# leejet/stable-diffusion.cpp

Measured on AMD Instinct MI355X. Metric: denoise it/s (image-iterations/s: cond+uncond UNet forwards per image per step), higher is better.
Workload: dtype f16; 1 GPU; sd15 UNet 512x512, cfg 7 (cond+uncond), f16 weights, batch 8/GPU, Euler-A step; global_batch=8, flash_attn=True, hip_graph=1, cfg_pair_in_one_graph=True, device_resident_sampler=True

## Files before the change

include/ggml-mi355x.h:

```cpp
#ifndef GGML_MI355X_H
#define GGML_MI355X_H

#include "ggml-abi.h"

#ifdef __cplusplus
extern "C" {
#endif

#define GGML_MI355X_API __attribute__((visibility("default")))

GGML_MI355X_API ggml_backend_reg_t ggml_backend_init(void);
GGML_MI355X_API int ggml_backend_score(void);
GGML_MI355X_API ggml_backend_reg_t ggml_backend_mi355x_reg(void);
GGML_MI355X_API int ggml_backend_mi355x_get_device_count(void);

struct ggml_backend_mi355x_stats {
    int64_t graphs_computed;
    int64_t plans_built;
    int64_t nodes_seen;
    int64_t kernels_planned;
    int64_t kernels_launched;
    int64_t fused_conv;
    int64_t fused_conv_bounced;
    int64_t fused_linear;
// ... 34 lines not shown
    int64_t fused_concat_gn;
    int64_t fused_conv_scale;
    int64_t view_graphs;
    int64_t plans_evicted;
    int64_t hoisted_mod_linears;
    int64_t view_external_nodes;
    int64_t qinloop_linears;
    int64_t flash_out_alias;
    int64_t flash_slice_images;
    int64_t flash_short_launches;
    int64_t flash_qb2_launches;
    int64_t flash_mslot_launches;
    int64_t flash_generic_launches;
    int64_t fused_gn_epilogue;
    int64_t fused_tile_merge;
};
GGML_MI355X_API void ggml_backend_mi355x_get_stats(struct ggml_backend_mi355x_stats* out);
GGML_MI355X_API int ggml_backend_mi355x_resolve_enums(const char* (*op_name)(int), const char* (*unary_op_name)(int), const char* (*type_name)(int));
GGML_MI355X_API const char* ggml_backend_mi355x_enum_status(void);
GGML_MI355X_API void ggml_backend_mi355x_get_enum_maps(uint8_t* ops256, uint8_t* unary256);
struct ggml_backend_mi355x_kernel_timing {
    char kernel[96];
    int64_t launches;
    double total_ms;
    double total_flops;
    double total_bytes;
    int32_t bound;
    int32_t family;
};
GGML_MI355X_API void ggml_backend_mi355x_kernel_timing_enable(int enable);
// ... 29 lines not shown
```

stable-diffusion.cpp_amd/__init__.py:

```python
from __future__ import annotations

import ctypes as C
import os
from pathlib import Path

import numpy as np

PKG_DIR = Path(__file__).resolve().parent
ROOT = PKG_DIR.parent
LIB_DIR = PKG_DIR / "lib"
HOST_LIB = Path(os.environ.get("SDCPP_HOST_LIB", str(LIB_DIR / "libsdcpp-host.so")))
BACKEND_LIB = Path(os.environ.get("SDCPP_BACKEND_LIB", str(LIB_DIR / "libggml-mi355x.so")))

F32, F16, Q4_0, Q8_0, I32, BF16 = 0, 1, 2, 8, 26, 30
TYPE_SIZE = {F32: 4, F16: 2, BF16: 2, I32: 4}

SD15, SDXL, SD15_TINY, SDXL_TINY, SD35_LARGE, SD35_TINY, FLUX_DEV, FLUX_TINY, SD35_WIDE2, FLUX_WIDE1, SD3M_TINY, SD35_WIDE8, FLUX_WIDE8 = 0, 1, 2, 3, 4, 5, 6, 7, 8, 9, 10, 11, 12
PAIR_EXCHANGE_FN = C.CFUNCTYPE(C.c_bool, C.c_void_p, C.c_int64, C.c_void_p, C.c_void_p)
EVAL_CALLBACK_FN = C.CFUNCTYPE(C.c_bool, C.c_void_p, C.c_bool, C.c_void_p)
EULER, EULER_A, HEUN, DPM2, DPMPP2S_A, DPMPP2M, DPMPP2Mv2, IPNDM, IPNDM_V, LCM, DDIM_TRAILING = range(11)
TCD, RES_MULTISTEP, RES_2S, ER_SDE, EULER_CFG_PP, EULER_A_CFG_PP, EULER_GE, DPMPP2M_SDE, DPMPP2M_SDE_BT, LMS = range(11, 21)
SAMPLE_METHOD_DEFAULT = 21
SCHED_DISCRETE, SCHED_KARRAS, SCHED_EXPONENTIAL, SCHED_AYS, SCHED_GITS, SCHED_SGM_UNIFORM, SCHED_SIMPLE, SCHED_SMOOTHSTEP, SCHED_KL_OPTIMAL, SCHED_LCM = range(10)
SCHED_BONG_TANGENT, SCHED_FLUX, SCHED_BETA, SCHEDULER_DEFAULT = 10, 14, 15, 16
# ... 337 lines not shown
    _loaded_plugins.add(p)


def load_mi355x_backend() -> None:
    if not BACKEND_LIB.exists():
        raise EngineError(f"{BACKEND_LIB} missing — the HIP backend was not built")
    load_backend(BACKEND_LIB)
    names = devices()
    if not any(n.upper().startswith("MI355X") for n in names):
        raise EngineError(f"libggml-mi355x.so loaded but exposes no MI355X device (devices: {names}); is a gfx950 GPU visible?")


_BACKEND_STAT_FIELDS = ("graphs_computed plans_built nodes_seen kernels_planned kernels_launched fused_conv fused_conv_bounced fused_linear "
                        "fused_norm fused_geglu fused_attention generic_matmul swizzled_weight_bytes graph_replays fused_linear_geglu "
                        "split_k_gemms head_major_gemms fused_modulate fused_gate fused_gelu fused_rope fused_concat_heads qgemv_linears fused_chan_add fused_proj_tokens gemm_attention fused_q16 split_k_inlaunch qgemm16_linears fgemv_linears fused_presilu fused_sibling_linears hoisted_kv_linears window_convs hoisted_emb_linears fused_rows16 fused_joint_qkv jit_images fused_cat_rows16 fused_gn_stats fused_ln_reduce redirect_fallbacks fused_concat_gn fused_conv_scale view_graphs plans_evicted hoisted_mod_linears view_external_nodes qinloop_linears flash_out_alias flash_slice_images "
                        "flash_short_launches flash_qb2_launches flash_mslot_launches flash_generic_launches fused_gn_epilogue fused_tile_merge").split()


class BackendStats(C.Structure):
    _fields_ = [(n, C.c_int64) for n in _BACKEND_STAT_FIELDS]


_backend_cdll = None


def _backend() -> C.CDLL:
    global _backend_cdll
    if _backend_cdll is None:
        load_mi355x_backend()
        _backend_cdll = C.CDLL(str(BACKEND_LIB))
        _backend_cdll.ggml_backend_mi355x_get_stats.argtypes = [C.POINTER(BackendStats)]
# ... 740 lines not shown
```

stable-diffusion.cpp_amd/csrc/backend/planner.cpp:

```cpp
#include "planner.h"

#include <atomic>
#include <cstddef>
#include <cstdio>
#include <cstdlib>
#include <cstring>
#include <functional>
#include <memory>
#include <mutex>
#include <string>
#include <algorithm>
#include <map>
#include <unordered_map>
#include <unordered_set>
#include <vector>

#include "kernels.h"
#include "ktime.h"

namespace mi355x {

static uint8_t g_opmap[256];
static uint8_t g_unmap[256];
static bool g_opmap_init = [] {
// ... 94 lines not shown
    return true;
}
void planner_get_op_maps(uint8_t* ops256, uint8_t* unary256) {
    if (ops256) memcpy(ops256, g_opmap, 256);
    if (unary256) memcpy(unary256, g_unmap, 256);
}

namespace {

constexpr size_t N_STATS = sizeof(ggml_backend_mi355x_stats) / sizeof(int64_t);
static_assert(N_STATS * sizeof(int64_t) == sizeof(ggml_backend_mi355x_stats), "ggml_backend_mi355x_stats: int64_t fields only");
std::atomic<int64_t> g_stat_counters[N_STATS];
#define STAT(field) g_stat_counters[offsetof(ggml_backend_mi355x_stats, field) / sizeof(int64_t)]

struct Options {
    std::atomic<int> fusion{1}, mfma_gemm{1}, hip_graph{1}, flash_pattern{1}, fuse_modulate{1}, fuse_gate{1}, fuse_gelu{1}, fuse_rope{1}, fuse_concat_heads{1}, qgemv{1}, fuse_chan_add{1}, fuse_proj_tokens{1}, fuse_q16{1}, qgemm16{1}, fgemv{1}, fuse_siblings{1}, hoist_kv{1}, hoist_emb{1}, fuse_rows16{0}, fuse_cat_rows16{1}, fuse_joint_qkv{1}, jit_qimages{4096}, fuse_gn_stats{1}, fuse_ln_reduce{1}, relax_res_overlap{1}, fuse_split_gelu{1}, fuse_concat_gn{1}, fuse_gn_tokens{1}, fuse_linear_nchw{1}, fuse_conv_scale{1}, ignore_use_counts{0}, plan_cache_cap{512}, hoist_mod{1}, fuse_flash_slices{1}, fuse_act_pack{1}, fuse_gn_epilogue{1}, fuse_tile_merge{1};
} g_opt;

using Step = std::function<void(hipStream_t)>;

struct Plan {
    int n_nodes = 0;
    uint64_t check = 0;
    size_t arena_needed = 0;
    std::vector<Step> steps;
    hipGraphExec_t graph_exec = nullptr;
    bool graph_failed         = false;
    int64_t runs              = 0;
    uint64_t last_use         = 0;
};

// ... 299 lines not shown
        Epilogue ep;
        int hd, hH, hL;
    };
    std::vector<HmLaunch> hm_group;
    std::unordered_map<const ggml_tensor*, size_t> moved;
    struct MovedEmb {
        size_t off;
        int64_t ld, M, N;
    };
    std::unordered_map<const ggml_tensor*, MovedEmb> moved_emb;
    struct GnPre {
        size_t off;
        const float *w, *b;
        int groups;
        float eps;
    };
    std::unordered_map<const ggml_tensor*, GnPre> gn_pre;
    std::unordered_map<const ggml_tensor*, size_t> gn_rec;
    struct LnPre {
        size_t off;
        const float *w, *b;
        float eps;
    };
    std::unordered_map<const ggml_tensor*, LnPre> ln_pre;
    struct Cat16 {
        size_t off;
        int64_t ld;
        bool written[2];
    };
    struct Cat16Part {
// ... 209 lines not shown
                    mul = sc;
                } else {
                    if (!(xop(cn) == GGML_OP_IM2COL && cn->src[1] == gi.node(k) && conv_im2col_fast_ok(gi, c))) return false;
                    if (n_real > 0 && mul != 1.f) return false;
                }
            } else {
                if (!(xop(cn) == GGML_OP_MUL_MAT && strip_reshape(cn->src[1]) == t && linear_fast_ok(cn))) return false;
            }
            ++n_real;
        }
    }
    if (mul_out) *mul_out = mul;
    return n_real > 0;
}

bool linear_fast_ok(const ggml_tensor* n) {
    const ggml_tensor* w = n->src[0];
    const ggml_tensor* x = n->src[1];
    if (!g_opt.mfma_gemm) return false;
    if (!is_static_weight(w) || !is_f32(x) || !is_f32(n)) return false;
    if (!(w->type == GGML_TYPE_F16 || w->type == GGML_TYPE_F32 || w->type == GGML_TYPE_BF16 || w->type == GGML_TYPE_Q8_0 || w->type == GGML_TYPE_Q4_0)) return false;
    if (w->ne[2] != 1 || w->ne[3] != 1 || !contig(w)) return false;
    if (x->nb[0] != 4 || x->ne[0] % 4 != 0 || x->nb[1] % 16 != 0 || !aligned16(x->data)) return false;
    if (x->ne[2] > 1 && x->nb[2] != x->nb[1] * (size_t)x->ne[1]) {
        if (x->ne[3] != 1 || x->nb[2] % 16 != 0) return false;
    }
    if (x->ne[3] > 1 && x->nb[3] != x->nb[2] * (size_t)x->ne[2]) return false;
    if (!contig(n)) return false;
    return true;
}
// ... 1043 lines not shown
        int r = gi.sole(last);
        if (r >= 0 && !gi.done[r] && xop(gi.node(r)) == GGML_OP_ADD && gi.only_noops_between(last, r, chain)) {
            const ggml_tensor* a     = gi.node(r);
            const ggml_tensor* other = a->src[0] == gi.node(last) ? a->src[1] : (a->src[1] == gi.node(last) ? a->src[0] : nullptr);
            if (other && is_f32(other) && contig(other) && contig(a) && ggml_abi_same_shape(other, a) && ggml_abi_same_shape(out, a) && gi.idx(other) < i &&
                (other->data == a->data || !overlaps(a->data, ob, other->data, ob))) {
                ep.residual = (const float*)other->data;
                chain.push_back(r);
                last = r;
            }
        }
    }
    float* final_dst = (float*)gi.node(last)->data;
    const int ks = KW, st_ = s0, pd = p0;
    Builder::GnPre gnp{0, nullptr, nullptr, 0, 0.f};
    if (g_opt.fuse_gn_stats && token_major_out < 0) {
        const ggml_tensor* res = gi.node(last);
        for (int k : gi.consumers[last]) {
            if (gnp.groups) break;
            const ggml_tensor* g = gi.node(k);
            if (xop(g) != GGML_OP_GROUP_NORM || g->src[0] != res || gi.done[k]) continue;
            const int j1 = gi.sole(k);
            if (j1 < 0 || xop(gi.node(j1)) != GGML_OP_MUL || gi.node(j1)->src[0] != g || !bias_like_chan(gi.node(j1)->src[1], OC)) break;
            const int j2 = gi.sole(j1);
            if (j2 < 0 || xop(gi.node(j2)) != GGML_OP_ADD || gi.node(j2)->src[0] != gi.node(j1) || !bias_like_chan(gi.node(j2)->src[1], OC)) break;
            const int64_t ohw = res->ne[0] * res->ne[1];
            if (!splitk_reduce_gn_supported(ohw, OC, N, g->op_params[0])) break;
            gnp = Builder::GnPre{0, (const float*)gi.node(j1)->src[1]->data, (const float*)gi.node(j2)->src[1]->data, g->op_params[0], ggml_abi_op_param_f32(g, 1)};
        }
    }
    const bool rec_want = g_opt.fuse_gn_epilogue && g_opt.fusion && token_major_out < 0 && feeds_group_norm(gi, last);
    auto gn_register = [&](int S) -> bool {
        if (S <= 1 || !gnp.groups) return false;
        if ((((uintptr_t)final_dst | (uintptr_t)ep.residual) & 15) != 0) return false;
        gnp.off                    = B.alloc((size_t)N * OC * 4 * 2);
        B.gn_pre[gi.node(last)]    = gnp;
        STAT(fused_gn_stats)++;
        return true;
    };
    auto gn_fill = [](Epilogue& e, const Builder::GnPre& g, char* arena, int64_t nc) {
        e.gn_scale  = (float*)(arena + g.off);
        e.gn_shift  = e.gn_scale + nc;
        e.gn_w      = g.w;
        e.gn_b      = g.b;
        e.gn_groups = g.groups;
        e.gn_eps    = g.eps;
    };
    const bool ups_in = B.ups.find(xs) != B.ups.end();
    const int w3S     = (token_major_out < 0) ? conv3w_plan(x->ne[0], x->ne[1], IC, N, OC, ks, st_, ups_in) : 0;
    const void* swz   = get_swz_conv(B.P, ker, s, w3S > 0);
    if (!swz) return false;
    const ggml_tensor* src = xs;
    bool upscale           = false;
    auto ui                = B.ups.find(xs);
    if (ui != B.ups.end()) {
        src     = ui->second;
        upscale = true;
    }
    const int64_t SW = src->ne[0], SH = src->ne[1];
    auto it = B.packed.find(src);
    if (it != B.packed.end() && it->second.nhwc && it->second.mul != pre_mul) {
// ... 77 lines not shown
    const size_t off = pk.off;
    const float* tp  = (const float*)t->data;
    B.emit([=](hipStream_t st) { launch_pack_rows_f16(st, P->arena + off, tp, N * HW, C, C); });
    B.packed[xr] = pk;
    return true;
}

bool plan_group_norm(Builder& B, int i, hipStream_t, std::vector<int>& chain) {
    GInfo& gi            = B.gi;
    const ggml_tensor* n = gi.node(i);
    const ggml_tensor* x = n->src[0];
    if (!is_f32(x) || !contig(x) || !contig(n)) return false;
    const int groups = n->op_params[0];
    const float eps  = ggml_abi_op_param_f32(n, 1);
    const int64_t hw = x->ne[0] * x->ne[1], C = x->ne[2], N = x->ne[3];
    const float *w = nullptr, *b = nullptr;
    bool silu = false;
    chain.push_back(i);
    int last = i;
    if (g_opt.fusion) {
        int j1 = gi.sole(i);
        if (j1 >= 0 && xop(gi.node(j1)) == GGML_OP_MUL && gi.node(j1)->src[0] == n && bias_like_chan(gi.node(j1)->src[1], C) && gi.node(j1)->data == n->data &&
            gi.only_noops_between(i, j1, chain)) {
            int j2 = gi.sole(j1);
            if (j2 >= 0 && xop(gi.node(j2)) == GGML_OP_ADD && gi.node(j2)->src[0] == gi.node(j1) && bias_like_chan(gi.node(j2)->src[1], C) &&
                gi.node(j2)->data == n->data && gi.only_noops_between(j1, j2, chain)) {
                w = (const float*)gi.node(j1)->src[1]->data;
                b = (const float*)gi.node(j2)->src[1]->data;
                chain.push_back(j1);
                chain.push_back(j2);
                last   = j2;
                int j3 = gi.sole(j2);
                if (j3 >= 0 && xop(gi.node(j3)) == GGML_OP_UNARY && xunary(gi.node(j3)) == GGML_UNARY_OP_SILU && gi.node(j3)->data == n->data &&
                    gi.only_noops_between(j2, j3, chain)) {
                    silu = true;
                    chain.push_back(j3);
                    last = j3;
                }
            }
        }
    }
    float* dst      = (float*)n->data;
    const float* xp = (const float*)x->data;
    int tok_cont = -1;
    if (g_opt.fusion && g_opt.fuse_gn_tokens && w && !silu) {
        const int jp = gi.sole(last);
        const ggml_tensor* pt = jp >= 0 ? gi.node(jp) : nullptr;
        if (pt && xop(pt) == GGML_OP_PERMUTE && pt->src[0] == gi.node(last) && pt->op_params[0] == 1 && pt->op_params[1] == 2 && pt->op_params[2] == 0 && pt->op_params[3] == 3) {
            const int jc = gi.sole(jp);
            const ggml_tensor* ct = jc >= 0 ? gi.node(jc) : nullptr;
            if (ct && xop(ct) == GGML_OP_CONT && ct->src[0] == pt && is_f32(ct) && contig(ct) && ct->ne[0] == C && !(ct->flags & GGML_TENSOR_FLAG_OUTPUT) && all_consumers_gemm16(gi, jc, false)) {
                std::vector<int> c2 = chain;
                c2.push_back(jp);
                c2.push_back(jc);
                if (gi.only_noops_between(last, jc, c2)) tok_cont = jc;
            }
        }
    }
    if (tok_cont >= 0) {
        Planner* P       = B.P;
        const auto pre   = B.gn_pre.find(x);
        const bool have  = pre != B.gn_pre.end() && pre->second.w == w && pre->second.b == b && pre->second.groups == groups && pre->second.eps == eps;
        const size_t so  = have ? pre->second.off : B.alloc((size_t)N * C * 4 * 2);
        const size_t off = B.alloc((size_t)N * hw * rup64(C) * 2);
        const auto rec   = B.gn_rec.find(x);
        const bool byrec = !have && g_opt.fuse_gn_epilogue && rec != B.gn_rec.end();
        const size_t ro  = byrec ? rec->second : 0;
        const int gsp    = (have || byrec) ? 0 : gn_stats_split(hw, C, N, groups);
        const size_t po  = gsp ? B.alloc((size_t)N * groups * gsp * 2 * 4) : 0;
        if (byrec) STAT(fused_gn_epilogue)++;
        B.emit([=](hipStream_t st) {
            float* sc = (float*)(P->arena + so);
            float* sh = sc + N * C;
            if (byrec) launch_gn_finalize(st, sc, sh, (const GnRec*)(P->arena + ro), nullptr, hw, C, C, N, groups, eps, w, b);
            else if (!have) launch_gn_stats(st, sc, sh, xp, hw, C, N, groups, eps, w, b, nullptr, 0, gsp ? (float*)(P->arena + po) : nullptr);
            launch_nchw_to_nhwc_f16(st, P->arena + off, xp, hw, C, N, sc, sh, false);
        });
        chain.push_back(gi.sole(last));
        chain.push_back(tok_cont);
        B.packed[gi.node(tok_cont)] = Packed{off, rup64(C), false};
        STAT(fused_norm)++;
        STAT(fused_proj_tokens)++;
        return true;
    }
    float conv_mul = 1.f;
    if (w && all_consumers_gemm16(gi, last, true, &conv_mul)) {
        Planner* P          = B.P;
        const auto pre      = B.gn_pre.find(x);
        const bool have     = pre != B.gn_pre.end() && pre->second.w == w && pre->second.b == b && pre->second.groups == groups && pre->second.eps == eps;
        const size_t so     = have ? pre->second.off : B.alloc((size_t)N * C * 4 * 2);
        const size_t off    = B.alloc((size_t)N * hw * rup64(C) * 2);
        const auto rec      = B.gn_rec.find(x);
        const bool byrec    = !have && g_opt.fuse_gn_epilogue && rec != B.gn_rec.end();
        const size_t ro     = byrec ? rec->second : 0;
        const int gsp       = (have || byrec) ? 0 : gn_stats_split(hw, C, N, groups);
        const size_t po     = gsp ? B.alloc((size_t)N * groups * gsp * 2 * 4) : 0;
        if (byrec) STAT(fused_gn_epilogue)++;
        B.emit([=](hipStream_t st) {
            float* sc = (float*)(P->arena + so);
            float* sh = sc + N * C;
            if (byrec) launch_gn_finalize(st, sc, sh, (const GnRec*)(P->arena + ro), nullptr, hw, C, C, N, groups, eps, w, b);
            else if (!have) launch_gn_stats(st, sc, sh, xp, hw, C, N, groups, eps, w, b, nullptr, 0, gsp ? (float*)(P->arena + po) : nullptr);
            launch_nchw_to_nhwc_f16(st, P->arena + off, xp, hw, C, N, sc, sh, silu, nullptr, 0, nullptr, conv_mul);
        });
// ... 1838 lines not shown
    {"t320_linear_max_split", nullptr, gemm16_set_t320_linear_max_split},
    OPT(qgemv),
    OPT(fuse_q16),
    {"streamk", nullptr, gemm16_set_streamk},
    {"geglu16", nullptr, gemm16_set_geglu16},
    {"bn64_max_tiles", nullptr, gemm16_set_bn64_max},
    {"conv3w_prio", nullptr, conv3w_set_prio},
    {"t256p_min_nt_sk", nullptr, gemm16_set_t256p_min_nt_sk},
    {"t256p_min_tiles_sk", nullptr, gemm16_set_t256p_min_tiles_sk},
    {"conv3w", nullptr, conv3w_set},
    OPT(hoist_emb),
    OPT(fuse_rows16),
    OPT(fuse_cat_rows16),
    OPT(fuse_gn_stats),
    OPT(fuse_gn_epilogue),
    OPT(fuse_tile_merge),
    OPT(fuse_joint_qkv),
    OPT(fuse_ln_reduce),
    OPT(jit_qimages),
    {"qinloop_min_rows", nullptr, gemm16_set_qinloop_min_rows},
    OPT(fuse_flash_slices),
    {"gemm16_t192p", nullptr, gemm16_set_t192p},
    {"conv3w_min_blocks", nullptr, conv3w_set_min_blocks},
    {"conv3w_min_blocks_deep", nullptr, conv3w_set_min_blocks_deep},
    {"gemm16_bn64", nullptr, gemm16_set_bn64},
    OPT(qgemm16),
    {"qgemv_max_rows", nullptr, qgemv_set_max_rows},
    OPT(fgemv),
    OPT(fuse_siblings),
    OPT(hoist_kv),
// ... 57 lines not shown
```

stable-diffusion.cpp_amd/csrc/kernels/gemm16.hip:

```cpp
#include <atomic>
#include <cstdio>
#include <cstdlib>
#include <mutex>
#include <type_traits>
#include <utility>
#include <vector>
#include "device_utils.h"
#include "kernels.h"
#include "ktime.h"
#include "g16_common.h"

namespace mi355x {

template <int BM, int BN, bool CONV, int BK, int NST, int WR, int WC, int PIPE = 0, bool SK = false, int QT = 0>
__global__ __launch_bounds__(WR * WC * 64, PIPE ? 2 : 2) void k_gemm16(G16Args g) {
    static_assert(!SK || (PIPE == 1 && !CONV), "stream-K is written for the pipelined Linear tiles");
    static_assert(QT == 0 || ((QT == 8 || QT == 4) && PIPE == 1 && !CONV && !SK && BM == 256 && (BN == 256 || BN == 192) && WR * WC == 8), "in-loop dequantisation: pipelined 256 x 256 / 256 x 192 Linear tiles");
    constexpr int NW  = WR * WC;
    constexpr int RB  = BM / WR / 32;
    constexpr int CB  = BN / WC / 32;
    static_assert(RB * WR * 32 == BM && CB * WC * 32 == BN, "tile must split into 32x32 blocks per wave");
    constexpr int ROWB   = BK * 2;
    constexpr int SLOTS  = ROWB / 16;
    constexpr int RPP    = 1024 / ROWB;
// ... 1295 lines not shown
            for (int j = 0; j < W; ++j) v[j] += chan_add[nimg * chan_ld + (i - nimg * C) + j];
        } else {
            const int64_t pc = i / inner, nimg = pc / C;
            const float b    = chan_add[nimg * chan_ld + (pc - nimg * C)];
#pragma unroll
            for (int j = 0; j < W; ++j) v[j] += b;
        }
    }
    if (residual) {
#pragma unroll
        for (int j = 0; j < W; ++j) v[j] += residual[i + j];
    }
#pragma unroll
    for (int j = 0; j < W; ++j) dst[i + j] = v[j];
}
template <int NT, int NV>
__global__ __launch_bounds__(NT) void k_splitk_reduce_gn(float* __restrict__ dst, const float* __restrict__ ws, int S, int64_t slab, int64_t hw, int C, int groups, int cpg,
                                                         const float* __restrict__ bias, const float* residual, const float* __restrict__ chan_add, int64_t chan_ld, float eps,
                                                         const float* __restrict__ gw, const float* __restrict__ gb, float* __restrict__ scale, float* __restrict__ shift) {
    __shared__ float scratch[2 * (NT / 64)];
    const int gidx = blockIdx.x % groups, n = blockIdx.x / groups;
    const int c0   = gidx * cpg;
    const int64_t cnt = (int64_t)cpg * hw, base = ((int64_t)n * C + c0) * hw, n4 = cnt / 4;
    float4 v[NV];
    float s = 0.f, dummy = 0.f;
#pragma unroll
    for (int j = 0; j < NV; ++j) {
        const int64_t i4 = threadIdx.x + (int64_t)NT * j;
        v[j]             = make_float4(0.f, 0.f, 0.f, 0.f);
        if (i4 < n4) {
            const int64_t e = i4 * 4, i = base + e;
            float4 a        = make_float4(0.f, 0.f, 0.f, 0.f);
            for (int sl = 0; sl < S; ++sl) {
                const float4 t = *(const float4*)(ws + sl * slab + i);
                a.x += t.x; a.y += t.y; a.z += t.z; a.w += t.w;
            }
// ... 18 lines not shown
    block_sum2<NT / 64>(s, dummy, scratch);
    const float mean = s / (float)cnt;
    float q = 0.f;
#pragma unroll
    for (int j = 0; j < NV; ++j) {
        if (threadIdx.x + (int64_t)NT * j < n4) {
            const float a = v[j].x - mean, bb = v[j].y - mean, c = v[j].z - mean, d = v[j].w - mean;
            q += (a * a + bb * bb) + (c * c + d * d);
        }
    }
    dummy = 0.f;
    block_sum2<NT / 64>(q, dummy, scratch);
    const float rstd = rsqrtf(q / (float)cnt + eps);
    for (int c = c0 + threadIdx.x; c < c0 + cpg; c += NT) {
        const float sc            = (gw ? gw[c] : 1.f) * rstd;
        scale[(int64_t)n * C + c] = sc;
        shift[(int64_t)n * C + c] = (gb ? gb[c] : 0.f) - mean * sc;
    }
}
bool splitk_reduce_gn_supported(int64_t hw, int64_t C, int64_t N, int groups) {
    if (groups <= 0 || C % groups != 0 || hw % 4 != 0 || N * groups < 256) return false;
    return (C / groups) * hw <= 4 * 1024 * 16;
}
static void launch_splitk_reduce_gn(hipStream_t s, float* dst, const float* ws, int S, int64_t hw, int64_t C, int64_t N, const Epilogue& e) {
    const int groups = e.gn_groups, cpg = (int)(C / groups);
    const int64_t cnt = (int64_t)cpg * hw, n = hw * C * N;
    const int64_t chan_ld = e.chan_ld > 0 ? e.chan_ld : C;
    KScope ks_(s, KF_SPLITK, 0.0, (double)n * 4.0 * (S + 1 + (e.residual ? 1 : 0)));
    const unsigned grid = (unsigned)(N * groups);
#define SKGN(NT_, NV_) k_splitk_reduce_gn<NT_, NV_><<<grid, NT_, 0, s>>>(dst, ws, S, n, hw, (int)C, groups, cpg, e.bias, e.residual, e.chan_add, chan_ld, e.gn_eps, e.gn_w, e.gn_b, e.gn_scale, e.gn_shift)
    if (cnt <= 4 * 256 * 4)
        SKGN(256, 4);
    else if (cnt <= 4 * 1024 * 4)
        SKGN(1024, 4);
    else
        SKGN(1024, 16);
#undef SKGN
}

static void launch_splitk_reduce(hipStream_t s, float* dst, const float* ws, int S, int64_t n, const float* bias, int64_t inner, int64_t C, const float* residual,
                                 const float* chan_add = nullptr, int64_t chan_ld = 0) {
    if (chan_ld <= 0) chan_ld = C;
    KScope ks_(s, KF_SPLITK, 0.0, (double)n * 4.0 * (S + 1));
    const bool v4 = n % 4 == 0 && (inner % 4 == 0 || (inner == 1 && C % 4 == 0)) && (((uintptr_t)dst | (uintptr_t)ws | (uintptr_t)residual) & 15) == 0;
    if (v4)
// ... 123 lines not shown
    return z;
}

void gemm16_init() { (void)zero_page(); }
const _Float16* gemm16_zero_page() { return zero_page(); }
[[noreturn]] static void g16_gn_contract_violation() {
    fprintf(stderr, "ggml-mi355x: split-K reduce asked for GroupNorm statistics on a shape / alignment it does not serve\n");
    abort();
}
void launch_splitk_reduce_conv(hipStream_t s, float* dst, const float* ws, int S, int64_t n, const float* bias, int64_t inner, int64_t C, const float* residual,
                               const float* chan_add, int64_t chan_ld) {
    launch_splitk_reduce(s, dst, ws, S, n, bias, inner, C, residual, chan_add, chan_ld);
}
void launch_splitk_reduce_conv_gn(hipStream_t s, float* dst, const float* ws, int S, int64_t hw, int64_t C, int64_t N, const Epilogue& e) {
    const bool gn_ok = (((uintptr_t)dst | (uintptr_t)ws | (uintptr_t)e.residual) & 15) == 0 && splitk_reduce_gn_supported(hw, C, N, e.gn_groups);
    if (e.gn_scale && !gn_ok) g16_gn_contract_violation();
    if (e.gn_scale)
        launch_splitk_reduce_gn(s, dst, ws, S, hw, C, N, e);
    else
        launch_splitk_reduce(s, dst, ws, S, hw * C * N, e.bias, hw, C, e.residual, e.chan_add, e.chan_ld);
}

static bool g16_trace() {
    static const bool on = getenv("GGML_MI355X_TRACE") != nullptr;
    return on;
}
static void g16_check_epi(const Epilogue& e) {
    if (e.act >= 0) {
        fprintf(stderr, "ggml-mi355x: gemm16 kernels have no fused activation (act=%d requested)\n", e.act);
        abort();
    }
// ... 234 lines not shown
    }
    const bool bn64 = OC <= 64;
    const double conv_bytes = (double)N * H * W * g.ICp * 2.0 + (double)g.ICp * ksize * ksize * rup64(OC, 128) * 2.0 + (double)g.R * OC * 4.0 * (e.residual ? 2.0 : 1.0);
    if (g16_trace())
        fprintf(stderr, "G16 conv rows=%lld K=%lld M=%lld res=%d ks=%d s=%d ups=%d hw=%lldx%lld ic=%lld\n", (long long)g.R, (long long)g.ICp * ksize * ksize, (long long)OC,
                e.residual ? 1 : 0, ksize, stride, g.UPS, (long long)W, (long long)H, (long long)IC);
    if (bn64) {
        g.ncol_tiles = (int)((OC + 63) / 64);
        g16_launch<64, true>(s, g, g.R, 2.0 * g.R * IC * ksize * ksize * OC, conv_bytes);
    } else {
        g.ncol_tiles = (int)((OC + 127) / 128);
        g16_launch<128, true>(s, g, g.R, 2.0 * g.R * IC * ksize * ksize * OC, conv_bytes);
    }
    if (S > 1 && !inker) {
        const bool gn_ok = (((uintptr_t)dst | (uintptr_t)splitk_ws | (uintptr_t)e.residual) & 15) == 0 && splitk_reduce_gn_supported(g.OHOW, OC, N, e.gn_groups);
        if (e.gn_scale && !gn_ok) g16_gn_contract_violation();
        if (e.gn_scale)
            launch_splitk_reduce_gn(s, dst, splitk_ws, S, g.OHOW, OC, N, e);
        else
            launch_splitk_reduce(s, dst, splitk_ws, S, g.R * OC, e.bias, g.OHOW, OC, e.residual, e.chan_add, e.chan_ld);
    }
}

__global__ void k_pack_rows_f16(_Float16* __restrict__ dst, const float* __restrict__ xin, int64_t R, int K, int Kp, int64_t xs, int64_t L, int64_t bs) {
    const int64_t n8 = R * (Kp / 8);
    for (int64_t i = blockIdx.x * (int64_t)blockDim.x + threadIdx.x; i < n8; i += (int64_t)gridDim.x * blockDim.x) {
        const int64_t r = i / (Kp / 8);
        const int k0    = (int)(i - r * (Kp / 8)) * 8;
        const float* x  = xin + (r / L) * bs + (r % L) * xs - r * xs;
        half8_t h;
        if (k0 + 8 <= K) {
// ... 650 lines not shown
```

stable-diffusion.cpp_amd/csrc/kernels/kernels.h:

```cpp
#pragma once
#include <hip/hip_runtime.h>
#include <stddef.h>
#include <stdint.h>

namespace mi355x {

struct View4 {
    const void* data;
    int64_t ne[4];
    int64_t nb[4];
    int type;
};

enum BinOp { BIN_ADD = 0, BIN_SUB = 1, BIN_MUL = 2, BIN_DIV = 3 };
enum UnOp { UN_SILU = 0, UN_GELU = 1, UN_GELU_QUICK = 2, UN_SIGMOID = 3, UN_TANH = 4, UN_RELU = 5, UN_NEG = 6, UN_EXP = 7 };

void launch_binary(hipStream_t s, BinOp op, void* dst, const int64_t dnb[4], const View4& a, const View4& b);
constexpr int TILE_MERGE_MAX = 32;
struct TileMergeTile {
    int x, y, w, h;
    int64_t src;
    int64_t wx, wy;
};
struct TileMergeArgs {
// ... 53 lines not shown
constexpr int GN_REC_CHUNK = 256;

struct Epilogue {
    const float* bias     = nullptr;
    const float* residual = nullptr;
    const float* chan_add = nullptr;
    int64_t chan_ld       = 0;
    float scale           = 1.0f;
    int act               = -1;
    float* gn_scale       = nullptr;
    float* gn_shift       = nullptr;
    const float* gn_w     = nullptr;
    const float* gn_b     = nullptr;
    int gn_groups         = 0;
    float gn_eps          = 0.f;
    GnRec* gn_rec         = nullptr;
    void* ln_dst16        = nullptr;
    const float* ln_w     = nullptr;
    const float* ln_b     = nullptr;
    float ln_eps          = 0.f;
    const float* gate     = nullptr;
    int gate_L            = 0;
    int gelu              = 0;
    int64_t split_col     = 0;
    void* split_dst16     = nullptr;
    int64_t split_ldd16   = 0;
    int qtype             = 0;
    int64_t qrow_bytes    = 0;
    int64_t a_run_L       = 0;
    int64_t a_run_S       = 0;
// ... 16 lines not shown
void gemm16_set_ln16_rows(int v);
void gemm16_set_tail_split(int v);
void gemm16_set_bn64(int v);
void gemm16_set_variant(int v);
void launch_gemm16_linear(hipStream_t s, float* dst, void* dst16, int64_t ldd16, const void* a16, int64_t lda, const void* wswz, int64_t rows,
                          int64_t K, int64_t M, int64_t ldd, const Epilogue& ep, int hm_d = 0, int hm_H = 0, int hm_L = 0, float* splitk_ws = nullptr, int* splitk_cnt = nullptr, int splitk_S = 0);
void launch_gemm16_linear_multi(hipStream_t s, int n, float* const* dst, void* const* dst16, const void* a16, int64_t lda, const void* const* wswz, int64_t rows,
                               int64_t K, int64_t M, const float* const* bias, float scale, int hm_d, int hm_H, int hm_L);
void launch_gemm16_linear_geglu(hipStream_t s, void* dst16, const void* a16, int64_t lda, const void* wswz_geglu, int64_t rows, int64_t K, int64_t M,
                                const float* bias, float* splitk_ws = nullptr, int* splitk_cnt = nullptr, int splitk_S = 0, int geglu_mode = 1);
int gemm16_geglu_mode(int64_t rows, int64_t M, int64_t K);
void gemm16_set_bn64_max(int v);
void gemm16_set_geglu16(int v);
int gemm16_split_k(int64_t rows, int64_t M, int64_t K, bool conv);
bool splitk_reduce_gn_supported(int64_t hw, int64_t C, int64_t N, int groups);
bool splitk_reduce_ln_supported(int64_t rows, int64_t M);
void gemm16_set_t320_linear_max_split(int v);
struct G16SplitPlan {
    int S;
    bool inkernel;
    size_t ws_bytes;
    int tiles;
};
G16SplitPlan gemm16_split_plan(int64_t rows, int64_t M, int64_t K, bool conv, bool plain_out, bool geglu = false);
void gemm16_set_splitk_inkernel(int v);
void gemm16_set_splitk_in_target(int v);
void launch_gemm16_conv(hipStream_t s, float* dst, const void* x16_nhwc, const void* wswz, int64_t W, int64_t H, int64_t IC, int64_t N, int64_t OC,
                        int ksize, int stride, int pad, bool upscale2x, const Epilogue& ep, float* splitk_ws = nullptr, int* splitk_cnt = nullptr, int splitk_S = 0);
bool gemm16_conv_gn_rec_supported(int64_t OHOW, int64_t N, int64_t OC, int64_t ICp, int ksize);
int conv3w_plan(int64_t W, int64_t H, int64_t IC, int64_t N, int64_t OC, int ksize, int stride, bool upscale2x, int* bn_out = nullptr);
// ... 71 lines not shown
```

Before: 374.6 it/s.

## Fuse GroupNorm apply and f16 NHWC pack into split-K conv reduce kernel

When a split-K conv feeds a GroupNorm (+affine, optional SiLU) whose consumers are all gemm16 convs, the split-K reduce kernel now also applies the norm and writes the packed f16 NHWC operand image. It transposes through LDS to do this. The GroupNorm node then just reuses that packed image instead of launching its own apply/pack kernel. This removes one kernel launch and a full re-read of the f32 activation per fused GroupNorm. The cost is more LDS use and a block-index swizzle in the reduce kernel, which can lower its occupancy.

Measured after the change: 376.0 it/s, median of 6. No clear change (+0.4%).

```diff
diff --git a/include/ggml-mi355x.h b/include/ggml-mi355x.h
--- a/include/ggml-mi355x.h
+++ b/include/ggml-mi355x.h
@@ -72,6 +72,7 @@
     int64_t flash_generic_launches;
     int64_t fused_gn_epilogue;
     int64_t fused_tile_merge;
+    int64_t fused_gn_reduce_apply;
 };
 GGML_MI355X_API void ggml_backend_mi355x_get_stats(struct ggml_backend_mi355x_stats* out);
 GGML_MI355X_API int ggml_backend_mi355x_resolve_enums(const char* (*op_name)(int), const char* (*unary_op_name)(int), const char* (*type_name)(int));
diff --git a/stable-diffusion.cpp_amd/__init__.py b/stable-diffusion.cpp_amd/__init__.py
--- a/stable-diffusion.cpp_amd/__init__.py
+++ b/stable-diffusion.cpp_amd/__init__.py
@@ -375,7 +375,7 @@
 _BACKEND_STAT_FIELDS = ("graphs_computed plans_built nodes_seen kernels_planned kernels_launched fused_conv fused_conv_bounced fused_linear "
                         "fused_norm fused_geglu fused_attention generic_matmul swizzled_weight_bytes graph_replays fused_linear_geglu "
                         "split_k_gemms head_major_gemms fused_modulate fused_gate fused_gelu fused_rope fused_concat_heads qgemv_linears fused_chan_add fused_proj_tokens gemm_attention fused_q16 split_k_inlaunch qgemm16_linears fgemv_linears fused_presilu fused_sibling_linears hoisted_kv_linears window_convs hoisted_emb_linears fused_rows16 fused_joint_qkv jit_images fused_cat_rows16 fused_gn_stats fused_ln_reduce redirect_fallbacks fused_concat_gn fused_conv_scale view_graphs plans_evicted hoisted_mod_linears view_external_nodes qinloop_linears flash_out_alias flash_slice_images "
-                        "flash_short_launches flash_qb2_launches flash_mslot_launches flash_generic_launches fused_gn_epilogue fused_tile_merge").split()
+                        "flash_short_launches flash_qb2_launches flash_mslot_launches flash_generic_launches fused_gn_epilogue fused_tile_merge fused_gn_reduce_apply").split()
 
 
 class BackendStats(C.Structure):
diff --git a/stable-diffusion.cpp_amd/csrc/backend/planner.cpp b/stable-diffusion.cpp_amd/csrc/backend/planner.cpp
--- a/stable-diffusion.cpp_amd/csrc/backend/planner.cpp
+++ b/stable-diffusion.cpp_amd/csrc/backend/planner.cpp
@@ -132,7 +132,7 @@
 #define STAT(field) g_stat_counters[offsetof(ggml_backend_mi355x_stats, field) / sizeof(int64_t)]
 
 struct Options {
-    std::atomic<int> fusion{1}, mfma_gemm{1}, hip_graph{1}, flash_pattern{1}, fuse_modulate{1}, fuse_gate{1}, fuse_gelu{1}, fuse_rope{1}, fuse_concat_heads{1}, qgemv{1}, fuse_chan_add{1}, fuse_proj_tokens{1}, fuse_q16{1}, qgemm16{1}, fgemv{1}, fuse_siblings{1}, hoist_kv{1}, hoist_emb{1}, fuse_rows16{0}, fuse_cat_rows16{1}, fuse_joint_qkv{1}, jit_qimages{4096}, fuse_gn_stats{1}, fuse_ln_reduce{1}, relax_res_overlap{1}, fuse_split_gelu{1}, fuse_concat_gn{1}, fuse_gn_tokens{1}, fuse_linear_nchw{1}, fuse_conv_scale{1}, ignore_use_counts{0}, plan_cache_cap{512}, hoist_mod{1}, fuse_flash_slices{1}, fuse_act_pack{1}, fuse_gn_epilogue{1}, fuse_tile_merge{1};
+    std::atomic<int> fusion{1}, mfma_gemm{1}, hip_graph{1}, flash_pattern{1}, fuse_modulate{1}, fuse_gate{1}, fuse_gelu{1}, fuse_rope{1}, fuse_concat_heads{1}, qgemv{1}, fuse_chan_add{1}, fuse_proj_tokens{1}, fuse_q16{1}, qgemm16{1}, fgemv{1}, fuse_siblings{1}, hoist_kv{1}, hoist_emb{1}, fuse_rows16{0}, fuse_cat_rows16{1}, fuse_joint_qkv{1}, jit_qimages{4096}, fuse_gn_stats{1}, fuse_ln_reduce{1}, relax_res_overlap{1}, fuse_split_gelu{1}, fuse_concat_gn{1}, fuse_gn_tokens{1}, fuse_linear_nchw{1}, fuse_conv_scale{1}, ignore_use_counts{0}, plan_cache_cap{512}, hoist_mod{1}, fuse_flash_slices{1}, fuse_act_pack{1}, fuse_gn_epilogue{1}, fuse_tile_merge{1}, fuse_gn_reduce_apply{1};
 } g_opt;
 
 using Step = std::function<void(hipStream_t)>;
@@ -462,6 +462,10 @@
         const float *w, *b;
         int groups;
         float eps;
+        bool img       = false;
+        size_t img_off = 0;
+        int img_act    = 0;
+        float img_mul  = 1.f;
     };
     std::unordered_map<const ggml_tensor*, GnPre> gn_pre;
     std::unordered_map<const ggml_tensor*, size_t> gn_rec;
@@ -701,6 +705,62 @@
     return n_real > 0;
 }
 
+struct GnChain {
+    const float *w = nullptr, *b = nullptr;
+    bool silu = false;
+    int last  = -1;
+    std::vector<int> chain;
+    int tok_cont  = -1;
+    bool conv_img = false;
+    float conv_mul = 1.f;
+};
+GnChain gn_chain_match(const GInfo& gi, int i) {
+    GnChain m;
+    const ggml_tensor* n = gi.node(i);
+    const int64_t C      = n->src[0]->ne[2];
+    m.chain.push_back(i);
+    m.last = i;
+    if (g_opt.fusion) {
+        int j1 = gi.sole(i);
+        if (j1 >= 0 && xop(gi.node(j1)) == GGML_OP_MUL && gi.node(j1)->src[0] == n && bias_like_chan(gi.node(j1)->src[1], C) && gi.node(j1)->data == n->data &&
+            gi.only_noops_between(i, j1, m.chain)) {
+            int j2 = gi.sole(j1);
+            if (j2 >= 0 && xop(gi.node(j2)) == GGML_OP_ADD && gi.node(j2)->src[0] == gi.node(j1) && bias_like_chan(gi.node(j2)->src[1], C) &&
+                gi.node(j2)->data == n->data && gi.only_noops_between(j1, j2, m.chain)) {
+                m.w = (const float*)gi.node(j1)->src[1]->data;
+                m.b = (const float*)gi.node(j2)->src[1]->data;
+                m.chain.push_back(j1);
+                m.chain.push_back(j2);
+                m.last = j2;
+                int j3 = gi.sole(j2);
+                if (j3 >= 0 && xop(gi.node(j3)) == GGML_OP_UNARY && xunary(gi.node(j3)) == GGML_UNARY_OP_SILU && gi.node(j3)->data == n->data &&
+                    gi.only_noops_between(j2, j3, m.chain)) {
+                    m.silu = true;
+                    m.chain.push_back(j3);
+                    m.last = j3;
+                }
+            }
+        }
+    }
+    if (g_opt.fusion && g_opt.fuse_gn_tokens && m.w && !m.silu) {
+        const int jp = gi.sole(m.last);
+        const ggml_tensor* pt = jp >= 0 ? gi.node(jp) : nullptr;
+        if (pt && xop(pt) == GGML_OP_PERMUTE && pt->src[0] == gi.node(m.last) && pt->op_params[0] == 1 && pt->op_params[1] == 2 && pt->op_params[2] == 0 && pt->op_params[3] == 3) {
+            const int jc = gi.sole(jp);
+            const ggml_tensor* ct = jc >= 0 ? gi.node(jc) : nullptr;
+            if (ct && xop(ct) == GGML_OP_CONT && ct->src[0] == pt && is_f32(ct) && contig(ct) && ct->ne[0] == C && !(ct->flags & GGML_TENSOR_FLAG_OUTPUT) && all_consumers_gemm16(gi, jc, false)) {
+                std::vector<int> c2 = m.chain;
+                c2.push_back(jp);
+                c2.push_back(jc);
+                if (gi.only_noops_between(m.last, jc, c2)) m.tok_cont = jc;
+            }
+        }
+    }
+    if (m.tok_cont < 0 && m.w) m.conv_img = all_consumers_gemm16(gi, m.last, true, &m.conv_mul);
+    if (!m.conv_img) m.conv_mul = 1.f;
+    return m;
+}
+
 bool linear_fast_ok(const ggml_tensor* n) {
     const ggml_tensor* w = n->src[0];
     const ggml_tensor* x = n->src[1];
@@ -1774,6 +1834,7 @@
     float* final_dst = (float*)gi.node(last)->data;
     const int ks = KW, st_ = s0, pd = p0;
     Builder::GnPre gnp{0, nullptr, nullptr, 0, 0.f};
+    int gn_node = -1;
     if (g_opt.fuse_gn_stats && token_major_out < 0) {
         const ggml_tensor* res = gi.node(last);
         for (int k : gi.consumers[last]) {
@@ -1787,6 +1848,7 @@
             const int64_t ohw = res->ne[0] * res->ne[1];
             if (!splitk_reduce_gn_supported(ohw, OC, N, g->op_params[0])) break;
             gnp = Builder::GnPre{0, (const float*)gi.node(j1)->src[1]->data, (const float*)gi.node(j2)->src[1]->data, g->op_params[0], ggml_abi_op_param_f32(g, 1)};
+            gn_node = k;
         }
     }
     const bool rec_want = g_opt.fuse_gn_epilogue && g_opt.fusion && token_major_out < 0 && feeds_group_norm(gi, last);
@@ -1794,6 +1856,18 @@
         if (S <= 1 || !gnp.groups) return false;
         if ((((uintptr_t)final_dst | (uintptr_t)ep.residual) & 15) != 0) return false;
         gnp.off                    = B.alloc((size_t)N * OC * 4 * 2);
+        const ggml_tensor* res = gi.node(last);
+        const int64_t ohw      = res->ne[0] * res->ne[1];
+        if (g_opt.fuse_gn_reduce_apply && g_opt.fusion && gn_node >= 0 && splitk_reduce_gn_apply_supported(ohw, OC, N, gnp.groups)) {
+            const GnChain m = gn_chain_match(gi, gn_node);
+            if (m.conv_img && m.w == gnp.w && m.b == gnp.b) {
+                gnp.img     = true;
+                gnp.img_off = B.alloc((size_t)N * ohw * rup64(OC) * 2);
+                gnp.img_act = m.silu ? 1 : 0;
+                gnp.img_mul = m.conv_mul;
+                STAT(fused_gn_reduce_apply)++;
+            }
+        }
         B.gn_pre[gi.node(last)]    = gnp;
         STAT(fused_gn_stats)++;
         return true;
@@ -1805,6 +1879,11 @@
         e.gn_b      = g.b;
         e.gn_groups = g.groups;
         e.gn_eps    = g.eps;
+        if (g.img) {
+            e.gn_img16   = arena + g.img_off;
+            e.gn_img_act = g.img_act;
+            e.gn_img_mul = g.img_mul;
+        }
     };
     const bool ups_in = B.ups.find(xs) != B.ups.end();
     const int w3S     = (token_major_out < 0) ? conv3w_plan(x->ne[0], x->ne[1], IC, N, OC, ks, st_, ups_in) : 0;
@@ -1912,49 +1991,14 @@
     const int groups = n->op_params[0];
     const float eps  = ggml_abi_op_param_f32(n, 1);
     const int64_t hw = x->ne[0] * x->ne[1], C = x->ne[2], N = x->ne[3];
-    const float *w = nullptr, *b = nullptr;
-    bool silu = false;
-    chain.push_back(i);
-    int last = i;
-    if (g_opt.fusion) {
-        int j1 = gi.sole(i);
-        if (j1 >= 0 && xop(gi.node(j1)) == GGML_OP_MUL && gi.node(j1)->src[0] == n && bias_like_chan(gi.node(j1)->src[1], C) && gi.node(j1)->data == n->data &&
-            gi.only_noops_between(i, j1, chain)) {
-            int j2 = gi.sole(j1);
-            if (j2 >= 0 && xop(gi.node(j2)) == GGML_OP_ADD && gi.node(j2)->src[0] == gi.node(j1) && bias_like_chan(gi.node(j2)->src[1], C) &&
-                gi.node(j2)->data == n->data && gi.only_noops_between(j1, j2, chain)) {
-                w = (const float*)gi.node(j1)->src[1]->data;
-                b = (const float*)gi.node(j2)->src[1]->data;
-                chain.push_back(j1);
-                chain.push_back(j2);
-                last   = j2;
-                int j3 = gi.sole(j2);
-                if (j3 >= 0 && xop(gi.node(j3)) == GGML_OP_UNARY && xunary(gi.node(j3)) == GGML_UNARY_OP_SILU && gi.node(j3)->data == n->data &&
-                    gi.only_noops_between(j2, j3, chain)) {
-                    silu = true;
-                    chain.push_back(j3);
-                    last = j3;
-                }
-            }
-        }
-    }
+    const GnChain m = gn_chain_match(gi, i);
+    const float *w = m.w, *b = m.b;
+    const bool silu = m.silu;
+    const int last  = m.last;
+    chain.insert(chain.end(), m.chain.begin(), m.chain.end());
     float* dst      = (float*)n->data;
     const float* xp = (const float*)x->data;
-    int tok_cont = -1;
-    if (g_opt.fusion && g_opt.fuse_gn_tokens && w && !silu) {
-        const int jp = gi.sole(last);
-        const ggml_tensor* pt = jp >= 0 ? gi.node(jp) : nullptr;
-        if (pt && xop(pt) == GGML_OP_PERMUTE && pt->src[0] == gi.node(last) && pt->op_params[0] == 1 && pt->op_params[1] == 2 && pt->op_params[2] == 0 && pt->op_params[3] == 3) {
-            const int jc = gi.sole(jp);
-            const ggml_tensor* ct = jc >= 0 ? gi.node(jc) : nullptr;
-            if (ct && xop(ct) == GGML_OP_CONT && ct->src[0] == pt && is_f32(ct) && contig(ct) && ct->ne[0] == C && !(ct->flags & GGML_TENSOR_FLAG_OUTPUT) && all_consumers_gemm16(gi, jc, false)) {
-                std::vector<int> c2 = chain;
-                c2.push_back(jp);
-                c2.push_back(jc);
-                if (gi.only_noops_between(last, jc, c2)) tok_cont = jc;
-            }
-        }
-    }
+    const int tok_cont = m.tok_cont;
     if (tok_cont >= 0) {
         Planner* P       = B.P;
         const auto pre   = B.gn_pre.find(x);
@@ -1981,11 +2025,16 @@
         STAT(fused_proj_tokens)++;
         return true;
     }
-    float conv_mul = 1.f;
-    if (w && all_consumers_gemm16(gi, last, true, &conv_mul)) {
+    const float conv_mul = m.conv_mul;
+    if (m.conv_img) {
         Planner* P          = B.P;
         const auto pre      = B.gn_pre.find(x);
         const bool have     = pre != B.gn_pre.end() && pre->second.w == w && pre->second.b == b && pre->second.groups == groups && pre->second.eps == eps;
+        if (have && pre->second.img) {
+            B.packed[gi.node(last)] = Packed{pre->second.img_off, rup64(C), true, conv_mul};
+            STAT(fused_norm)++;
+            return true;
+        }
         const size_t so     = have ? pre->second.off : B.alloc((size_t)N * C * 4 * 2);
         const size_t off    = B.alloc((size_t)N * hw * rup64(C) * 2);
         const auto rec      = B.gn_rec.find(x);
@@ -3854,6 +3903,7 @@
     OPT(fuse_cat_rows16),
     OPT(fuse_gn_stats),
     OPT(fuse_gn_epilogue),
+    OPT(fuse_gn_reduce_apply),
     OPT(fuse_tile_merge),
     OPT(fuse_joint_qkv),
     OPT(fuse_ln_reduce),
diff --git a/stable-diffusion.cpp_amd/csrc/kernels/gemm16.hip b/stable-diffusion.cpp_amd/csrc/kernels/gemm16.hip
--- a/stable-diffusion.cpp_amd/csrc/kernels/gemm16.hip
+++ b/stable-diffusion.cpp_amd/csrc/kernels/gemm16.hip
@@ -1333,12 +1333,20 @@
 #pragma unroll
     for (int j = 0; j < W; ++j) dst[i + j] = v[j];
 }
-template <int NT, int NV>
+constexpr int GN_IMG_MAX_CPG = 128;
+constexpr int GN_IMG_PAD     = 4;
+template <int NT, int NV, bool IMG>
 __global__ __launch_bounds__(NT) void k_splitk_reduce_gn(float* __restrict__ dst, const float* __restrict__ ws, int S, int64_t slab, int64_t hw, int C, int groups, int cpg,
                                                          const float* __restrict__ bias, const float* residual, const float* __restrict__ chan_add, int64_t chan_ld, float eps,
-                                                         const float* __restrict__ gw, const float* __restrict__ gb, float* __restrict__ scale, float* __restrict__ shift) {
+                                                         const float* __restrict__ gw, const float* __restrict__ gb, float* __restrict__ scale, float* __restrict__ shift,
+                                                         _Float16* __restrict__ img = nullptr, int silu = 0, float post_mul = 1.f) {
     __shared__ float scratch[2 * (NT / 64)];
-    const int gidx = blockIdx.x % groups, n = blockIdx.x / groups;
+    constexpr int STAGE_HALFS = IMG ? (NT * NV * 4 < 32768 ? NT * NV * 4 : 32768) + GN_IMG_PAD * GN_IMG_MAX_CPG : 4;
+    __shared__ alignas(16) _Float16 st16[STAGE_HALFS];
+    __shared__ float tab[IMG ? 2 * GN_IMG_MAX_CPG : 1];
+    unsigned bid = blockIdx.x;
+    if (IMG && gridDim.x % 8 == 0) bid = (bid % 8) * (gridDim.x / 8) + bid / 8;
+    const int gidx = bid % groups, n = bid / groups;
     const int c0   = gidx * cpg;
     const int64_t cnt = (int64_t)cpg * hw, base = ((int64_t)n * C + c0) * hw, n4 = cnt / 4;
     float4 v[NV];
@@ -1387,21 +1395,85 @@
     const float rstd = rsqrtf(q / (float)cnt + eps);
     for (int c = c0 + threadIdx.x; c < c0 + cpg; c += NT) {
         const float sc            = (gw ? gw[c] : 1.f) * rstd;
+        const float sh            = (gb ? gb[c] : 0.f) - mean * sc;
         scale[(int64_t)n * C + c] = sc;
-        shift[(int64_t)n * C + c] = (gb ? gb[c] : 0.f) - mean * sc;
+        shift[(int64_t)n * C + c] = sh;
+        if (IMG) {
+            tab[c - c0]                  = sc;
+            tab[GN_IMG_MAX_CPG + c - c0] = sh;
+        }
+    }
+    if (IMG) {
+        __syncthreads();
+        const int ihw = (int)hw, rs = ihw + GN_IMG_PAD;
+#pragma unroll
+        for (int j = 0; j < NV; ++j) {
+            const int e = (threadIdx.x + NT * j) * 4;
+            if (e < (int)cnt) {
+                const int cl = e / ihw, p = e - cl * ihw;
+                const float sc = tab[cl], sh = tab[GN_IMG_MAX_CPG + cl];
+                const float a[4] = {v[j].x, v[j].y, v[j].z, v[j].w};
+                uint16_t h[4];
+#pragma unroll
+                for (int q = 0; q < 4; ++q) {
+                    float u = a[q] * sc + sh;
+                    if (silu == 1) u = act_apply<UN_SILU>(u);
+                    else if (silu == 2) u = act_apply<UN_RELU>(u);
+                    u *= post_mul;
+                    h[q] = __builtin_bit_cast(uint16_t, (_Float16)u);
+                }
+                *(uint2*)(st16 + cl * rs + p) = make_uint2((uint32_t)h[0] | ((uint32_t)h[1] << 16), (uint32_t)h[2] | ((uint32_t)h[3] << 16));
+            }
+        }
+        __syncthreads();
+        const int Cp = C;
+        const uint16_t* sg = (const uint16_t*)st16;
+        _Float16* dn       = img + (int64_t)n * hw * Cp + c0;
+        if ((cpg & 3) == 0) {
+            const int wpp = cpg / 4, nw = (int)cnt / 4;
+            for (int w = threadIdx.x; w < nw; w += NT) {
+                const int p = w / wpp, cw = w - p * wpp;
+                const uint16_t* q = sg + 4 * cw * rs + p;
+                *(uint2*)(dn + (int64_t)p * Cp + 4 * cw) = make_uint2((uint32_t)q[0] | ((uint32_t)q[rs] << 16), (uint32_t)q[2 * rs] | ((uint32_t)q[3 * rs] << 16));
+            }
+        } else {
+            const int wpp = cpg / 2, nw = (int)cnt / 2;
+            for (int w = threadIdx.x; w < nw; w += NT) {
+                const int p = w / wpp, cw = w - p * wpp;
+                const uint16_t* q = sg + 2 * cw * rs + p;
+                *(uint32_t*)(dn + (int64_t)p * Cp + 2 * cw) = (uint32_t)q[0] | ((uint32_t)q[rs] << 16);
+            }
+        }
     }
 }
 bool splitk_reduce_gn_supported(int64_t hw, int64_t C, int64_t N, int groups) {
     if (groups <= 0 || C % groups != 0 || hw % 4 != 0 || N * groups < 256) return false;
     return (C / groups) * hw <= 4 * 1024 * 16;
+}
+bool splitk_reduce_gn_apply_supported(int64_t hw, int64_t C, int64_t N, int groups) {
+    if (!splitk_reduce_gn_supported(hw, C, N, groups) || C % 64 != 0) return false;
+    const int64_t cpg = C / groups;
+    return cpg % 2 == 0 && cpg <= GN_IMG_MAX_CPG && cpg * hw * 2 <= 64 * 1024;
 }
 static void launch_splitk_reduce_gn(hipStream_t s, float* dst, const float* ws, int S, int64_t hw, int64_t C, int64_t N, const Epilogue& e) {
     const int groups = e.gn_groups, cpg = (int)(C / groups);
     const int64_t cnt = (int64_t)cpg * hw, n = hw * C * N;
     const int64_t chan_ld = e.chan_ld > 0 ? e.chan_ld : C;
-    KScope ks_(s, KF_SPLITK, 0.0, (double)n * 4.0 * (S + 1 + (e.residual ? 1 : 0)));
+    if (e.gn_img16 && (!splitk_reduce_gn_apply_supported(hw, C, N, groups) || ((uintptr_t)e.gn_img16 & 15) != 0)) {
+        fprintf(stderr, "ggml-mi355x: split-K reduce asked for a GroupNorm operand image on a shape / alignment it does not serve\n");
+        abort();
+    }
+    KScope ks_(s, KF_SPLITK, 0.0, (double)n * 4.0 * (S + 1 + (e.residual ? 1 : 0)) + (e.gn_img16 ? (double)n * 2.0 : 0.0));
     const unsigned grid = (unsigned)(N * groups);
-#define SKGN(NT_, NV_) k_splitk_reduce_gn<NT_, NV_><<<grid, NT_, 0, s>>>(dst, ws, S, n, hw, (int)C, groups, cpg, e.bias, e.residual, e.chan_add, chan_ld, e.gn_eps, e.gn_w, e.gn_b, e.gn_scale, e.gn_shift)
+#define SKGN(NT_, NV_)                                                                                                                                              \
+    do {                                                                                                                                                            \
+        if (e.gn_img16)                                                                                                                                             \
+            k_splitk_reduce_gn<NT_, NV_, true><<<grid, NT_, 0, s>>>(dst, ws, S, n, hw, (int)C, groups, cpg, e.bias, e.residual, e.chan_add, chan_ld, e.gn_eps, e.gn_w, \
+                                                                     e.gn_b, e.gn_scale, e.gn_shift, (_Float16*)e.gn_img16, e.gn_img_act, e.gn_img_mul);               \
+        else                                                                                                                                                        \
+            k_splitk_reduce_gn<NT_, NV_, false><<<grid, NT_, 0, s>>>(dst, ws, S, n, hw, (int)C, groups, cpg, e.bias, e.residual, e.chan_add, chan_ld, e.gn_eps, e.gn_w, \
+                                                                      e.gn_b, e.gn_scale, e.gn_shift);                                                                  \
+    } while (0)
     if (cnt <= 4 * 256 * 4)
         SKGN(256, 4);
     else if (cnt <= 4 * 1024 * 4)
@@ -1555,7 +1627,7 @@
 }
 void launch_splitk_reduce_conv_gn(hipStream_t s, float* dst, const float* ws, int S, int64_t hw, int64_t C, int64_t N, const Epilogue& e) {
     const bool gn_ok = (((uintptr_t)dst | (uintptr_t)ws | (uintptr_t)e.residual) & 15) == 0 && splitk_reduce_gn_supported(hw, C, N, e.gn_groups);
-    if (e.gn_scale && !gn_ok) g16_gn_contract_violation();
+    if ((e.gn_scale && !gn_ok) || (e.gn_img16 && !e.gn_scale)) g16_gn_contract_violation();
     if (e.gn_scale)
         launch_splitk_reduce_gn(s, dst, ws, S, hw, C, N, e);
     else
@@ -1820,7 +1892,7 @@
     }
     if (S > 1 && !inker) {
         const bool gn_ok = (((uintptr_t)dst | (uintptr_t)splitk_ws | (uintptr_t)e.residual) & 15) == 0 && splitk_reduce_gn_supported(g.OHOW, OC, N, e.gn_groups);
-        if (e.gn_scale && !gn_ok) g16_gn_contract_violation();
+        if ((e.gn_scale && !gn_ok) || (e.gn_img16 && !e.gn_scale)) g16_gn_contract_violation();
         if (e.gn_scale)
             launch_splitk_reduce_gn(s, dst, splitk_ws, S, g.OHOW, OC, N, e);
         else
diff --git a/stable-diffusion.cpp_amd/csrc/kernels/kernels.h b/stable-diffusion.cpp_amd/csrc/kernels/kernels.h
--- a/stable-diffusion.cpp_amd/csrc/kernels/kernels.h
+++ b/stable-diffusion.cpp_amd/csrc/kernels/kernels.h
@@ -91,6 +91,9 @@
     const float* gn_b     = nullptr;
     int gn_groups         = 0;
     float gn_eps          = 0.f;
+    void* gn_img16        = nullptr;
+    int gn_img_act        = 0;
+    float gn_img_mul      = 1.f;
     GnRec* gn_rec         = nullptr;
     void* ln_dst16        = nullptr;
     const float* ln_w     = nullptr;
@@ -137,6 +140,7 @@
 void gemm16_set_geglu16(int v);
 int gemm16_split_k(int64_t rows, int64_t M, int64_t K, bool conv);
 bool splitk_reduce_gn_supported(int64_t hw, int64_t C, int64_t N, int groups);
+bool splitk_reduce_gn_apply_supported(int64_t hw, int64_t C, int64_t N, int groups);
 bool splitk_reduce_ln_supported(int64_t rows, int64_t M);
 void gemm16_set_t320_linear_max_split(int v);
 struct G16SplitPlan {
```
